# RUCAIBox/RecBole-CDR

Hardware: AMD Instinct MI355X
Metric: training interactions/sec (higher is better)
Workload: dtype f32; 1 GPU; C5: EMCDR-BPR D=128, 50000000 users x 10000000 items/domain (union tables 71.7 GB fp32), step = source batch + target batch of 1048576 triples each per rank, fwd+bwd+row-wise adam; batch_per_domain_per_rank=1048576, k_neg=1, optimizer=rowwise-adam

## Files before the change

recbole-cdr_amd/csrc/cdr_step.hip:

```cpp
#include <cstdlib>
#include <cstring>
#include <string.h>
#include <rocprim/device/device_radix_sort.hpp>
#include <rocprim/device/device_scan.hpp>
#include <rocprim/iterator/counting_iterator.hpp>
#include <rocprim/iterator/transform_iterator.hpp>
#include "cdr_common.h"
#include "cdr_adam_math.h"
#include "cdr_loss_math.h"

namespace {

constexpr int kUnroll = 4;

#ifndef CDR_NORM_REC_FLOATS
#define CDR_NORM_REC_FLOATS 16
#endif
constexpr int kNormRecFloats = CDR_NORM_REC_FLOATS;
static_assert(kNormRecFloats == 16 || kNormRecFloats == 32, "a record is one 64-byte or one 128-byte burst");

template <int LPR>
__device__ __forceinline__ float sqnorm4(float4 a) {
    if constexpr (LPR >= 32) {
        return __builtin_fmaf(a.w, a.w, __builtin_fmaf(a.z, a.z, __builtin_fmaf(a.x, a.x, a.y * a.y)));
// ... 246 lines not shown
        out6[6] = (float)acc[0]; out6[7] = (float)acc[1]; out6[8] = (float)acc[2];
    }
}

__global__ void finish_sums_kernel(const float* __restrict__ sums3, int64_t B, float reg_weight, float* __restrict__ out6) {
    if (threadIdx.x == 0 && blockIdx.x == 0) {
        const float main_loss = sums3[0] / (float)B;
        const float nu = sqrtf(sums3[1]), ni = sqrtf(sums3[2]);
        out6[1] = main_loss; out6[2] = nu; out6[3] = ni;
        out6[0] = main_loss + reg_weight * ((nu + ni) / (float)B);
        out6[4] = embloss_coef(reg_weight, B, nu);
        out6[5] = embloss_coef(reg_weight, B, ni);
    }
}

__global__ __launch_bounds__(kBlock) void make_keys_kernel(const int64_t* __restrict__ ids0, int64_t n0,
                                                           const int64_t* __restrict__ ids1, int64_t n1,
                                                           uint32_t* __restrict__ keys, uint32_t* __restrict__ vals) {
    const int64_t n = n0 + n1, stride = (int64_t)gridDim.x * kBlock;
    for (int64_t e = (int64_t)blockIdx.x * kBlock + threadIdx.x; e < n; e += stride) {
        keys[e] = (uint32_t)(e < n0 ? ids0[e] : ids1[e - n0]);
        vals[e] = (uint32_t)e;
    }
}

constexpr int kLongSeg = 32;
constexpr int kPiece = 256;

struct seg_long { int64_t head, len, base; };
struct seg_piece { int64_t start; int64_t len; };

struct apply_hp { float lr, b1, b2, eps, wd, step_size, bc2_sqrt; const float* dev; };
#define HP_FROM_DEV(h) do { if ((h).dev) { (h).step_size = (h).dev[0]; (h).bc2_sqrt = (h).dev[1]; } } while (0)
// ... 202 lines not shown
        if (NC) norm_rec_store<LPR>(n2 + (int64_t)row * kNormRecFloats, group_sum<LPR>(sqnorm4<LPR>(wnew)), sub);
    }
}
template <int LPR, int OPT>
__global__ __launch_bounds__(kBlock) void seg_long_finish_kernel(float* __restrict__ W, float* __restrict__ Mo, float* __restrict__ Vo,
                                                                 int D, const uint32_t* __restrict__ keys,
                                                                 const float* __restrict__ reg_coef, apply_hp hp,
                                                                 const unsigned* __restrict__ counters,
                                                                 const seg_long* __restrict__ longs,
                                                                 const float* __restrict__ partial, const int* __restrict__ pcnt) {
    seg_long_finish_body<LPR, OPT>(W, Mo, Vo, D, keys, reg_coef, hp, counters, longs, partial, pcnt);
}

__global__ __launch_bounds__(kBlock) void make_keys2_kernel(const int64_t* __restrict__ a, int64_t na, const int64_t* __restrict__ b0,
                                                            int64_t nb0, const int64_t* __restrict__ b1, int64_t nb1, uint32_t key_base,
                                                            uint32_t* __restrict__ keys, uint32_t* __restrict__ vals) {
    const int64_t n = na + nb0 + nb1, stride = (int64_t)gridDim.x * kBlock;
    for (int64_t e = (int64_t)blockIdx.x * kBlock + threadIdx.x; e < n; e += stride) {
        if (e < na) { keys[e] = (uint32_t)a[e]; vals[e] = (uint32_t)e; }
        else {
            const int64_t o = e - na;
            keys[e] = key_base + (uint32_t)(o < nb0 ? b0[o] : b1[o - nb0]);
            vals[e] = (uint32_t)o;
        }
    }
}


struct tab_ptrs { float* W; float* M; float* V; };

template <int OPT>
__device__ __forceinline__ float4 upd_math(float4 w, float4& m, float4& v, float4 acc, float rc, const apply_hp& h) {
    float4 gr = make_float4(acc.x + rc * w.x, acc.y + rc * w.y, acc.z + rc * w.z, acc.w + rc * w.w);
    if (h.wd != 0.f) { gr.x += h.wd * w.x; gr.y += h.wd * w.y; gr.z += h.wd * w.z; gr.w += h.wd * w.w; }
    if (OPT == 0) return make_float4(w.x - h.lr * gr.x, w.y - h.lr * gr.y, w.z - h.lr * gr.z, w.w - h.lr * gr.w);
    m.x += (gr.x - m.x) * (1.0f - h.b1); m.y += (gr.y - m.y) * (1.0f - h.b1);
    m.z += (gr.z - m.z) * (1.0f - h.b1); m.w += (gr.w - m.w) * (1.0f - h.b1);
    v.x = h.b2 * v.x + (1.0f - h.b2) * gr.x * gr.x; v.y = h.b2 * v.y + (1.0f - h.b2) * gr.y * gr.y;
    v.z = h.b2 * v.z + (1.0f - h.b2) * gr.z * gr.z; v.w = h.b2 * v.w + (1.0f - h.b2) * gr.w * gr.w;
// ... 172 lines not shown
        __syncthreads();
        unsigned sA = wbase[0][wave] + pA - cA, sB = wbase[1][wave] + pB - cB;
#pragma unroll
        for (int j = 0; j < kFlagIT; ++j) {
            if ((hA >> j) & 1u) headsA[sA++] = (uint32_t)(q0 + j);
            if ((hB >> j) & 1u) headsB[sB++] = (uint32_t)(q0 + j - nA);
        }
        __syncthreads();
    }
}

__global__ __launch_bounds__(kBlock) void coef_finish_kernel(const double* __restrict__ partials, int nblocks, int64_t B,
                                                             float reg_weight, float* __restrict__ out9, int kmul = 1,
                                                             int64_t* __restrict__ step_u_dev = nullptr, int64_t* __restrict__ step_i_dev = nullptr,
                                                             float* __restrict__ hp_dev = nullptr, float lr = 0.f, float b1 = 0.f, float b2 = 0.f,
                                                             unsigned* __restrict__ zero4 = nullptr, const float* __restrict__ norms2 = nullptr) {
    __shared__ double smem[2 * (kBlock / 64)];
    if (zero4 && threadIdx.x >= 64 && threadIdx.x < 68) zero4[threadIdx.x - 64] = 0u;
    if (hp_dev && threadIdx.x < 2) {
        int64_t* c = threadIdx.x == 0 ? step_u_dev : step_i_dev;
        const int64_t st = c[0] + 1;
        c[0] = st;
        cdr_adam_hp((double)st, lr, b1, b2, hp_dev[2 * threadIdx.x], hp_dev[2 * threadIdx.x + 1]);
    }
    double acc[2] = {0.0, 0.0};
    sum_partials<2, kBlock>(partials, nblocks, acc, smem);
    if (threadIdx.x == 0) {
        if (norms2) { acc[0] = (double)norms2[0]; acc[1] = (double)norms2[1]; }
        const float nu = (float)sqrt((double)kmul * acc[0]), ni = (float)sqrt((double)kmul * acc[1]);
        out9[4] = (reg_weight != 0.f && nu > 0.f) ? (float)kmul * (reg_weight / ((float)B * nu)) : 0.f;
        out9[5] = (reg_weight != 0.f && ni > 0.f) ? (float)kmul * (reg_weight / ((float)B * ni)) : 0.f;
    }
}
// ... 604 lines not shown
template <int LPR>
__global__ __launch_bounds__(kBlock) void seg_piece_sum2_kernel(int D, dup_side a, dup_side b) {
    const dup_side& t = blockIdx.y ? b : a;
    if (t.counters == nullptr) return;
    seg_piece_sum_body<LPR, true>(D, t.perm, t.G, t.neg_start, t.reg_limit, nullptr, t.counters, t.pieces, t.partial, t.pcnt);
}
template <int LPR, int OPT, bool NC = false>
__global__ __launch_bounds__(kBlock) void seg_long_finish2_kernel(int D, dup_side a, dup_side b) {
    const dup_side& t = blockIdx.y ? b : a;
    if (t.counters == nullptr) return;
    seg_long_finish_body<LPR, OPT, NC>(t.W, t.M, t.V, D, t.keys, t.reg_coef, t.hp, t.counters, t.longs, t.partial, t.pcnt, t.n2);
}

__global__ __launch_bounds__(kBlock) void shard_keys_kernel(const int64_t* __restrict__ recv3, int64_t Bl, uint32_t G, unsigned lb,
                                                            uint32_t key_base, int64_t* __restrict__ u_loc, uint32_t* __restrict__ keys,
                                                            uint32_t* __restrict__ vals, unsigned* __restrict__ cnt) {
    if (blockIdx.x == 0 && threadIdx.x < 4) cnt[threadIdx.x] = 0u;
    for (int64_t t = (int64_t)blockIdx.x * kBlock + threadIdx.x; t < Bl; t += (int64_t)gridDim.x * kBlock) {
        const int64_t u = recv3[3 * t];
        const uint32_t p = (uint32_t)recv3[3 * t + 1], n = (uint32_t)recv3[3 * t + 2];
        u_loc[t] = u;
        keys[t] = (uint32_t)u; vals[t] = (uint32_t)t;
        keys[Bl + t] = key_base + (((p % G) << lb) | (p / G)); vals[Bl + t] = (uint32_t)t;
        keys[2 * Bl + t] = key_base + (((n % G) << lb) | (n / G)); vals[2 * Bl + t] = (uint32_t)(Bl + t);
    }
}

struct head_flag_op {
    const uint32_t* keys;
    __device__ uint32_t operator()(uint32_t q) const { return (q == 0u || keys[q] != keys[q - 1]) ? 1u : 0u; }
};
// ... 527 lines not shown
    CDR_LAUNCH_CHECK();
    triplet_finish_kernel<<<dim3(1), dim3(kBlock), 0, s>>>(ctx->partials, grid, B, out3);
    CDR_LAUNCH_CHECK();
    return CDR_OK;
}

extern "C" int cdr_loss_finish_sums(void* stream, const float* sums3, int64_t B_mean, float reg_weight, float* out6) {
    CDR_CHECK_ARG(sums3 && out6 && B_mean > 0);
    finish_sums_kernel<<<dim3(1), dim3(64), 0, (hipStream_t)stream>>>(sums3, B_mean, reg_weight, out6);
    CDR_LAUNCH_CHECK();
    return CDR_OK;
}

using big_sort_config = rocprim::radix_sort_config<
    rocprim::default_config, rocprim::default_config,
    rocprim::radix_sort_onesweep_config<rocprim::kernel_config<1024, 8>, rocprim::kernel_config<1024, 8>, 9,
                                        rocprim::block_radix_rank_algorithm::match>,
    (size_t)1 << 17>;
constexpr int64_t kBigSort = 1 << 18;

static inline hipError_t sort_pairs(void* tmp, size_t& tmp_bytes, const uint32_t* kin, uint32_t* kout, const uint32_t* vin, uint32_t* vout,
                                    size_t n, unsigned bits, hipStream_t s) {
    if ((int64_t)n >= kBigSort) return rocprim::radix_sort_pairs<big_sort_config>(tmp, tmp_bytes, kin, kout, vin, vout, n, 0u, bits, s);
    return rocprim::radix_sort_pairs(tmp, tmp_bytes, kin, kout, vin, vout, n, 0u, bits, s);
}

static inline unsigned bits_for(int64_t num_rows) {
    unsigned b = 1;
    while (b < 32 && ((int64_t)1 << b) < num_rows) ++b;
    return b;
}

namespace {

inline size_t up256(size_t b) { return (b + 255) & ~(size_t)255; }

struct heads_view {
    unsigned* cnt; uint32_t* headsA; uint32_t* headsB;
    heads_view(uint32_t* heads, int64_t n_a) : cnt((unsigned*)heads), headsA(heads + 4), headsB(headsA + (n_a / 2 + 1)) {}
    static int64_t words(int64_t n_a, int64_t n_b) { return 4 + (n_a / 2 + 1) + (n_b / 2 + 1); }
};

inline size_t count_list_bytes(int64_t B) {
    int64_t P = 1024;
    while (P < 3 * B) P <<= 1;
    return (size_t)(P + kListHdr) * sizeof(uint64_t);
// ... 24 lines not shown
        o_part = o_cnt + up256(sizeof(int) * piece_cap); bytes = o_part + sizeof(float) * (size_t)piece_cap * D;
    }
    void bind(char* base, dup_side& t) const {
        t.counters = (unsigned*)base; t.longs = (seg_long*)(base + o_long); t.pieces = (seg_piece*)(base + o_piece);
        t.pcnt = (int*)(base + o_cnt); t.partial = (float*)(base + o_part);
    }
};

}

extern "C" int cdr_sort_workspace_bytes(int64_t n, int64_t num_rows, size_t* bytes) {
    CDR_CHECK_ARG(bytes && n > 0 && num_rows > 0 && num_rows <= (int64_t)0xFFFFFFFFu && n <= (int64_t)0x7FFFFFFF);
    size_t tmp = 0;
    hipError_t e = sort_pairs(nullptr, tmp, nullptr, nullptr, nullptr, nullptr, (size_t)n, bits_for(num_rows), (hipStream_t)0);
    if (e != hipSuccess) { cdr_set_error("cdr_sort_workspace_bytes: %s", hipGetErrorString(e)); return (int)e; }
    *bytes = up256(tmp) + 2 * up256((size_t)n * sizeof(uint32_t));
    return CDR_OK;
}

template <class MakeKeys>
static int sort_ids_with(cdr_ctx* ctx, hipStream_t s, int64_t n, int64_t key_space, uint32_t* keys_sorted, uint32_t* perm, void* ws,
                         size_t ws_bytes, MakeKeys&& make_keys) {
    size_t need = 0;
    int rc = cdr_sort_workspace_bytes(n, key_space, &need);
    if (rc) return rc;
    CDR_CHECK_ARG(ws_bytes >= need);
    const size_t arr = up256((size_t)n * sizeof(uint32_t));
    uint32_t* keys_in = (uint32_t*)ws;
    uint32_t* vals_in = (uint32_t*)((char*)ws + arr);
    void* tmp = (char*)ws + 2 * arr;
    size_t tmp_bytes = ws_bytes - 2 * arr;
    cdr_time_scope ts(ctx, CDR_TAG_SORT, s);
    make_keys(keys_in, vals_in);
    CDR_LAUNCH_CHECK();
    CDR_HIP(sort_pairs(tmp, tmp_bytes, keys_in, keys_sorted, vals_in, perm, (size_t)n, bits_for(key_space), s));
    return CDR_OK;
}

extern "C" int cdr_sort_ids(cdr_ctx* ctx, void* stream, const int64_t* ids0, int64_t n0, const int64_t* ids1, int64_t n1,
                            int64_t num_rows, uint32_t* keys_sorted, uint32_t* perm, void* workspace,
                            size_t workspace_bytes) {
    const int64_t n = n0 + n1;
    CDR_CHECK_ARG(ids0 && n0 > 0 && (n1 == 0 || ids1) && keys_sorted && perm && workspace);
    hipStream_t s = (hipStream_t)stream;
    return sort_ids_with(ctx, s, n, num_rows, keys_sorted, perm, workspace, workspace_bytes, [&](uint32_t* keys_in, uint32_t* vals_in) {
        make_keys_kernel<<<dim3(grid_for(n, kBlock)), dim3(kBlock), 0, s>>>(ids0, n0, ids1, n1, keys_in, vals_in);
    });
}

extern "C" int cdr_sort_ids_two_tables(cdr_ctx* ctx, void* stream, const int64_t* ids_a, int64_t n_a, int64_t rows_a,
                                       const int64_t* ids_b0, int64_t n_b0, const int64_t* ids_b1, int64_t n_b1, int64_t rows_b,
                                       uint32_t* keys_sorted, uint32_t* perm, uint32_t* key_base_out, void* workspace,
                                       size_t workspace_bytes) {
    const int64_t n = n_a + n_b0 + n_b1;
    CDR_CHECK_ARG(ids_a && n_a > 0 && ids_b0 && n_b0 > 0 && (n_b1 == 0 || ids_b1) && keys_sorted && perm && key_base_out && workspace);
    CDR_CHECK_ARG(rows_a > 0 && rows_b > 0);
    const unsigned hb = two_table_bits(rows_a, rows_b);
    CDR_CHECK_ARG(hb < 31);
    const uint32_t key_base = 1u << hb;
    hipStream_t s = (hipStream_t)stream;
    int rc = sort_ids_with(ctx, s, n, (int64_t)key_base * 2, keys_sorted, perm, workspace, workspace_bytes, [&](uint32_t* keys_in, uint32_t* vals_in) {
        make_keys2_kernel<<<dim3(grid_for(n, kBlock)), dim3(kBlock), 0, s>>>(ids_a, n_a, ids_b0, n_b0, ids_b1, n_b1, key_base, keys_in, vals_in);
    });
    if (rc) return rc;
    *key_base_out = key_base;
    return CDR_OK;
}

extern "C" int cdr_rowwise_apply(cdr_ctx* ctx, void* stream, int opt, float* table, float* exp_avg, float* exp_avg_sq, int D,
                                 const uint32_t* keys_sorted, const uint32_t* perm, int64_t n, const float* G,
                                 int64_t neg_start, int64_t reg_limit, const float* reg_coef, float lr, float beta1,
                                 float beta2, float eps, float weight_decay, int64_t step, const int64_t* occ_ids, uint32_t key_base) {
    CDR_CHECK_ARG(table && keys_sorted && perm && G && n > 0);
    CDR_CHECK_ARG(D > 0 && (D & 3) == 0);
    CDR_CHECK_ARG(opt == 0 || (opt == 1 && exp_avg && exp_avg_sq && step > 0));
    hipStream_t s = (hipStream_t)stream;
    if (key_base) {
        table -= (int64_t)key_base * D;
        if (exp_avg) exp_avg -= (int64_t)key_base * D;
        if (exp_avg_sq) exp_avg_sq -= (int64_t)key_base * D;
    }
// ... 33 lines not shown
    return CDR_OK;
}

namespace {

struct step_tables { tab_ptrs TU, TI; apply_hp hu, hi; };
step_tables make_tables(int opt_user, float* user_tab, float* user_m, float* user_v, int64_t step_user, int opt_item, float* item_tab,
                        float* item_m, float* item_v, int64_t step_item, float lr, float beta1, float beta2, float eps, float wd) {
    return {{user_tab, user_m, user_v}, {item_tab, item_m, item_v}, make_hp(opt_user, lr, beta1, beta2, eps, wd, step_user),
            make_hp(opt_item, lr, beta1, beta2, eps, wd, step_item)};
}

int embloss_head(cdr_ctx* ctx, hipStream_t s, const float* user_tab, const float* item_tab, int D, const int64_t* uid, const int64_t* pid,
                 int64_t n_rows, int64_t B, int kmul, float reg_weight, float* out9, unsigned* cnt, int64_t* step_user_dev = nullptr,
                 int64_t* step_item_dev = nullptr, float* hp_dev = nullptr, float lr = 0.f, float beta1 = 0.f, float beta2 = 0.f,
                 const float* user_n2 = nullptr, const float* item_n2 = nullptr) {
    int ngrid = 0;
    if (reg_weight != 0.f) {
        const int lpr = cdr_lpr_for(D);
        ngrid = grid_for((n_rows + 7) / 8, kBlock / lpr);
        cdr_time_scope ts(ctx, CDR_TAG_BATCH_NORMS, s);
        if (user_n2 && item_n2) {
            DISPATCH_LPR(lpr, batch_norms_cached_kernel<L><<<dim3(ngrid), dim3(kBlock), 0, s>>>(user_n2, item_n2, uid, pid, n_rows, ctx->partials));
        } else {
            DISPATCH_LPR(lpr, batch_norms_kernel<L><<<dim3(ngrid), dim3(kBlock), 0, s>>>(user_tab, item_tab, D, uid, pid, n_rows, ctx->partials));
        }
        CDR_LAUNCH_CHECK();
    }
    coef_finish_kernel<<<dim3(1), dim3(kBlock), 0, s>>>(ctx->partials, ngrid, B, ngrid ? reg_weight : 0.f, out9, kmul, step_user_dev, step_item_dev, hp_dev,
                                                        lr, beta1, beta2, cnt);
    CDR_LAUNCH_CHECK();
    return CDR_OK;
}

int occ_flags(cdr_ctx* ctx, hipStream_t s, const uint32_t* keys, const uint32_t* perm, int64_t n_a, int64_t n, int fstride, uint8_t* flags,
              const heads_view& hv, bool stat = false) {
    cdr_time_scope ts(ctx, CDR_TAG_OCC_FLAGS, s);
    occ_flags_kernel<<<dim3(grid_for(n, kBlock * kFlagIT)), dim3(kBlock), 0, s>>>(keys, perm, n_a, n, fstride, flags, hv.headsA, hv.headsB, hv.cnt, stat);
    CDR_LAUNCH_CHECK();
    return CDR_OK;
}

struct dup_host { tab_ptrs T; const uint32_t* keys; const uint32_t* perm; int64_t n; const uint32_t* heads; const unsigned* nheads;
                  const float* G; int64_t neg_start, reg_limit; const float* reg_coef; apply_hp hp; uint32_t key_base;
                  float* out = nullptr; const uint32_t* uidx = nullptr; float* n2 = nullptr; };
// ... 119 lines not shown
        }
        CDR_LAUNCH_CHECK();
        coef_finish_kernel<<<dim3(1), dim3(kBlock), 0, s>>>(ctx->partials, reg_weight != 0.f ? ngrid : 0, B, reg_weight, out9, 1, step_user_dev, step_item_dev, hp_dev,
                                                            lr, beta1, beta2, hv.cnt);
        CDR_LAUNCH_CHECK();
        {
            cdr_time_scope ts(ctx, CDR_TAG_OCC_FLAGS, s);
            count_flags_kernel<<<dim3(grid_for(B, kBlock)), dim3(kBlock), 0, s>>>(uid, pid, nid, B, ctx->idc_user, ctx->idc_item, key_base, (uint32_t*)flags,
                                                                                 (uint64_t*)ctx->idc_list, hv.cnt);
            CDR_LAUNCH_CHECK();
            count_sort_kernel<<<dim3(kRankBlocks + 128), dim3(1024), 0, s>>>(uid, pid, nid, B, ctx->idc_user, ctx->idc_item, key_base,
                                                                                            (uint64_t*)ctx->idc_list, keys, perm, hv.headsA, hv.headsB, hv.cnt);
        }
        CDR_LAUNCH_CHECK();
    } else {
        rc = embloss_head(ctx, s, user_tab, item_tab, D, uid, pid, B, B, 1, reg_weight, out9, hv.cnt, step_user_dev, step_item_dev, hp_dev, lr, beta1, beta2,
                          NU, NI);
        if (rc) return rc;
        rc = cdr_sort_ids_two_tables(ctx, stream, uid, B, user_rows, pid, B, nid, B, item_rows, keys, perm, &key_base, sort_ws, sort_ws_bytes);
        if (rc) return rc;
        rc = occ_flags(ctx, s, keys, perm, B, 3 * B, 4, flags, hv, B <= kCountMaxB);
        if (rc) return rc;
    }
    step_tables T = make_tables(opt, user_tab, user_m, user_v, step_user, opt, item_tab, item_m, item_v, step_item, lr, beta1, beta2, eps, weight_decay);
    if (hp_dev && opt == 1) { T.hu.dev = hp_dev; T.hi.dev = hp_dev + 2; }
    static const int un = [] { const char* e = getenv("CDR_FWD_APPLY_UN"); return (e && e[0] == '2') ? 2 : 1; }();
    const int grid = grid_for((B + un - 1) / un, kBlock / lpr);
    {
        cdr_time_scope ts(ctx, CDR_TAG_BPR_FWD_APPLY, s);
        DISPATCH_LPR_OPT(lpr, opt, {
            constexpr int U2 = O == 1 ? 2 : 1;
            auto kern = cached ? (un == 2 ? bpr_fwd_apply_kernel<L, O, U2, false, false, true> : bpr_fwd_apply_kernel<L, O, 1, false, false, true>)
                               : (un == 2 ? bpr_fwd_apply_kernel<L, O, U2> : bpr_fwd_apply_kernel<L, O, 1>);
            kern<<<dim3(grid), dim3(kBlock), 0, s>>>(T.TU, T.TI, D, uid, pid, nid, (const uint32_t*)flags, B, gamma, 1.0f / (float)B, out9 + 4, T.hu, T.hi, GU, GP,
// ... 312 lines not shown
extern "C" int cdr_bpr_shard_plan(cdr_ctx* ctx, void* stream, const int64_t* recv3, int64_t Bl, int64_t user_rows, int64_t item_local_rows,
                                  int world, int64_t* u_loc, uint32_t* keys, uint32_t* perm, uint8_t* flags, uint32_t* heads,
                                  uint32_t* uidx, int64_t* uniq_local, int64_t* umap, int64_t* counts, int64_t* n_uniq, void* ws,
                                  size_t ws_bytes) {
    CDR_CHECK_ARG(ctx && recv3 && u_loc && keys && perm && flags && heads && uidx && uniq_local && umap && counts && n_uniq && ws);
    CDR_CHECK_ARG(Bl > 0 && 3 * Bl <= (int64_t)0x7FFFFFFF && ((uintptr_t)flags & 3) == 0);
    shard_bits kb;
    CDR_CHECK_ARG(shard_key_bits(user_rows, item_local_rows, world, kb) == CDR_OK);
    size_t scan_need = 0;
    int rc = shard_scan_bytes(Bl, &scan_need);
    if (rc) return rc;
    CDR_CHECK_ARG(ws_bytes >= scan_need);
    hipStream_t s = (hipStream_t)stream;
    const int64_t n = 3 * Bl;
    const heads_view hv(heads, Bl);
    rc = sort_ids_with(ctx, s, n, (int64_t)kb.key_base * 2, keys, perm, ws, ws_bytes, [&](uint32_t* keys_in, uint32_t* vals_in) {
        shard_keys_kernel<<<dim3(grid_for(Bl, kBlock)), dim3(kBlock), 0, s>>>(recv3, Bl, (uint32_t)world, kb.lb, kb.key_base, u_loc, keys_in, vals_in, hv.cnt);
    });
    if (rc) return rc;
    rc = occ_flags(ctx, s, keys, perm, Bl, n, 4, flags, hv);
    if (rc) return rc;
    const int64_t nB = 2 * Bl;
    const uint32_t* keysB = keys + Bl;
    const size_t arrB = up256((size_t)nB * sizeof(uint32_t));
    uint32_t* excl = (uint32_t*)ws;
    void* stmp = (char*)ws + arrB;
    size_t stmp_bytes = ws_bytes - arrB;
    CDR_HIP(rocprim::exclusive_scan(stmp, stmp_bytes, rocprim::make_transform_iterator(rocprim::make_counting_iterator<uint32_t>(0u), head_flag_op{keysB}),
                                    excl, 0u, (size_t)nB, rocprim::plus<uint32_t>(), s));
    shard_emit_kernel<<<dim3(grid_for(nB, kBlock)), dim3(kBlock), 0, s>>>(keysB, perm + Bl, excl, nB, world, kb.lb, kb.key_base, uidx, uniq_local, umap,
                                                                          counts, n_uniq);
    CDR_LAUNCH_CHECK();
// ... 112 lines not shown
        });
    }
    CDR_LAUNCH_CHECK();
    dup_host sides[2];
    make_sides(sides, T, keys, perm, hv, GU, GI, S, nI, nI, S, out9 + 4, out9 + 5, key_base);
    return finish_and_apply_dups(ctx, s, opt, D, sides, [&](unsigned* za, unsigned* zb) {
        step_finish_keep_kernel<<<dim3(1), dim3(kBlock), 0, s>>>(ctx->partials, grid, B, reg_weight, out9, za, zb);
    });
}

namespace {

__global__ __launch_bounds__(kBlock) void make_keys_pair_kernel(const int64_t* __restrict__ a0, int64_t na0, const int64_t* __restrict__ a1,
                                                                int64_t na1, const int64_t* __restrict__ b0, int64_t nb0,
                                                                const int64_t* __restrict__ b1, int64_t nb1, uint32_t key_base,
                                                                uint32_t* __restrict__ keys, uint32_t* __restrict__ vals) {
    const int64_t na = na0 + na1, n = na + nb0 + nb1, stride = (int64_t)gridDim.x * kBlock;
    for (int64_t e = (int64_t)blockIdx.x * kBlock + threadIdx.x; e < n; e += stride) {
        if (e < na) { keys[e] = (uint32_t)(e < na0 ? a0[e] : a1[e - na0]); vals[e] = (uint32_t)e; }
        else {
            const int64_t o = e - na;
            keys[e] = key_base + (uint32_t)(o < nb0 ? b0[o] : b1[o - nb0]);
            vals[e] = (uint32_t)o;
        }
    }
}

template <int LPR>
__global__ __launch_bounds__(kBlock) void pair_norms_kernel(const float* __restrict__ U, const float* __restrict__ I, int D,
                                                            const int64_t* __restrict__ su, const int64_t* __restrict__ si, int64_t Bs,
                                                            const int64_t* __restrict__ tu, const int64_t* __restrict__ ti, int64_t Bt,
// ... 180 lines not shown
    const float wreg_s = alpha * reg_s, wreg_t = (1.0f - alpha) * reg_t;
    const heads_view hv(heads, N);
    int ngrid = 0;
    if (wreg_s != 0.f || wreg_t != 0.f) {
        ngrid = grid_for((N + 7) / 8, kBlock / lpr);
        cdr_time_scope ts(ctx, CDR_TAG_BATCH_NORMS, s);
        DISPATCH_LPR(lpr, pair_norms_kernel<L><<<dim3(ngrid), dim3(kBlock), 0, s>>>(user_tab, item_tab, D, su, si, B_s, tu, ti, B_t, ctx->partials));
        CDR_LAUNCH_CHECK();
    }
    pair_coef_kernel<<<dim3(1), dim3(kBlock), 0, s>>>(ctx->partials, ngrid, B_s, B_t, wreg_s, wreg_t, out16, step_user_dev, step_item_dev,
                                                      opt == 1 ? hp_dev : nullptr, lr, beta1, beta2, hv.cnt);
    CDR_LAUNCH_CHECK();
    const unsigned hb = two_table_bits(user_rows, item_rows);
    CDR_CHECK_ARG(hb < 31);
    const uint32_t key_base = 1u << hb;
    int rc = sort_ids_with(ctx, s, 2 * N, (int64_t)key_base * 2, keys, perm, sort_ws, sort_ws_bytes, [&](uint32_t* keys_in, uint32_t* vals_in) {
        make_keys_pair_kernel<<<dim3(grid_for(2 * N, kBlock)), dim3(kBlock), 0, s>>>(su, B_s, tu, B_t, si, B_s, ti, B_t, key_base, keys_in, vals_in);
    });
    if (rc) return rc;
    rc = occ_flags(ctx, s, keys, perm, N, 2 * N, 4, flags, hv);
    if (rc) return rc;
    step_tables T = make_tables(opt, user_tab, user_m, user_v, 1, opt, item_tab, item_m, item_v, 1, lr, beta1, beta2, eps, weight_decay);
    if (opt == 1) { T.hu.dev = hp_dev; T.hi.dev = hp_dev + 2; }
    const int grid = grid_for(N, kBlock / lpr);
    {
        cdr_time_scope ts(ctx, CDR_TAG_POINT_FWD_GRAD, s);
        DISPATCH_LPR_OPT(lpr, opt, point_pair_fwd_apply_kernel<L, O><<<dim3(grid), dim3(kBlock), 0, s>>>(
                                       loss_kind, T.TU, T.TI, D, su, si, ys, B_s, tu, ti, yt, B_t, (const uint32_t*)flags, alpha / (float)B_s, (1.0f - alpha) / (float)B_t,
                                       out16 + 9, T.hu, T.hi, GU, GI, ctx->partials));
    }
    CDR_LAUNCH_CHECK();
    dup_host sides[2];
// ... 6 lines not shown
```

Baseline: 568.7 million interactions/s.

## Replace rocPRIM sort driver with own onesweep passes and fuse setup into key kernels

For large sorts with rocPRIM 4.2, the change stops calling rocPRIM's sort_pairs wrapper and launches rocPRIM's onesweep histogram, scan and pass device functions directly. The clearing of sort workspace state (lookback, block ids, counts) moves into the key-building kernels, or into the coefficient-finish kernel. On the two-table path, the digit histogram and its prefix scan are folded into the key-generation kernel. The aim is to drop memset, histogram and scan launches and one extra read of the keys per step. The price is reliance on rocPRIM detail internals tied to one version, plus more shared-memory atomics in the key kernel.

```diff
diff --git a/recbole-cdr_amd/csrc/cdr_step.hip b/recbole-cdr_amd/csrc/cdr_step.hip
--- a/recbole-cdr_amd/csrc/cdr_step.hip
+++ b/recbole-cdr_amd/csrc/cdr_step.hip
@@ -284,9 +284,16 @@
     }
 }
 
+__device__ __forceinline__ void sort_state_clear(uint32_t* __restrict__ zspan, int64_t zwords) {
+    if (!zspan) return;
+    for (int64_t i = (int64_t)blockIdx.x * blockDim.x + threadIdx.x; i < zwords; i += (int64_t)gridDim.x * blockDim.x) zspan[i] = 0u;
+}
+
 __global__ __launch_bounds__(kBlock) void make_keys_kernel(const int64_t* __restrict__ ids0, int64_t n0,
                                                            const int64_t* __restrict__ ids1, int64_t n1,
-                                                           uint32_t* __restrict__ keys, uint32_t* __restrict__ vals) {
+                                                           uint32_t* __restrict__ keys, uint32_t* __restrict__ vals,
+                                                           uint32_t* __restrict__ zspan, int64_t zwords) {
+    sort_state_clear(zspan, zwords);
     const int64_t n = n0 + n1, stride = (int64_t)gridDim.x * kBlock;
     for (int64_t e = (int64_t)blockIdx.x * kBlock + threadIdx.x; e < n; e += stride) {
         keys[e] = (uint32_t)(e < n0 ? ids0[e] : ids1[e - n0]);
@@ -519,7 +526,9 @@
 
 __global__ __launch_bounds__(kBlock) void make_keys2_kernel(const int64_t* __restrict__ a, int64_t na, const int64_t* __restrict__ b0,
                                                             int64_t nb0, const int64_t* __restrict__ b1, int64_t nb1, uint32_t key_base,
-                                                            uint32_t* __restrict__ keys, uint32_t* __restrict__ vals) {
+                                                            uint32_t* __restrict__ keys, uint32_t* __restrict__ vals,
+                                                            uint32_t* __restrict__ zspan, int64_t zwords) {
+    sort_state_clear(zspan, zwords);
     const int64_t n = na + nb0 + nb1, stride = (int64_t)gridDim.x * kBlock;
     for (int64_t e = (int64_t)blockIdx.x * kBlock + threadIdx.x; e < n; e += stride) {
         if (e < na) { keys[e] = (uint32_t)a[e]; vals[e] = (uint32_t)e; }
@@ -528,6 +537,64 @@
             keys[e] = key_base + (uint32_t)(o < nb0 ? b0[o] : b1[o - nb0]);
             vals[e] = (uint32_t)o;
         }
+    }
+}
+
+constexpr unsigned kSortBlock = 1024, kSortItems = 8, kSortRadixBits = 9, kSortRadix = 1u << kSortRadixBits;
+constexpr unsigned kSortMaxPlaces = (32 + kSortRadixBits - 1) / kSortRadixBits;
+using sort_offs_t = size_t;
+
+__global__ __launch_bounds__(kSortBlock) void make_keys2_offsets_kernel(const int64_t* __restrict__ a, int64_t na, const int64_t* __restrict__ b0,
+                                                                        int64_t nb0, const int64_t* __restrict__ b1, int64_t nb1,
+                                                                        uint32_t key_base, uint32_t* __restrict__ keys, uint32_t* __restrict__ vals,
+                                                                        uint32_t* __restrict__ zspan, int64_t zwords,
+                                                                        sort_offs_t* __restrict__ counts, unsigned* __restrict__ ticket, unsigned places) {
+    constexpr unsigned kStripes = 4;
+    __shared__ unsigned hist[kSortMaxPlaces * kSortRadix * kStripes];
+    sort_state_clear(zspan, zwords);
+    const unsigned tid = threadIdx.x, bins = places * kSortRadix;
+    for (unsigned i = tid; i < bins * kStripes; i += kSortBlock) hist[i] = 0u;
+    __syncthreads();
+    const unsigned stripe = tid % kStripes;
+    const int64_t n = na + nb0 + nb1, stride = (int64_t)gridDim.x * kSortBlock;
+    for (int64_t e = (int64_t)blockIdx.x * kSortBlock + tid; e < n; e += stride) {
+        uint32_t k, v;
+        if (e < na) { k = (uint32_t)a[e]; v = (uint32_t)e; }
+        else {
+            const int64_t o = e - na;
+            k = key_base + (uint32_t)(o < nb0 ? b0[o] : b1[o - nb0]);
+            v = (uint32_t)o;
+        }
+        keys[e] = k; vals[e] = v;
+        for (unsigned p = 0; p < places; ++p) {
+            const unsigned digit = (k >> (p * kSortRadixBits)) & (kSortRadix - 1u);
+            atomicAdd(&hist[(p * kSortRadix + digit) * kStripes + stripe], 1u);
+        }
+    }
+    __syncthreads();
+    for (unsigned i = tid; i < bins; i += kSortBlock) {
+        unsigned t = 0;
+#pragma unroll
+        for (unsigned j = 0; j < kStripes; ++j) t += hist[i * kStripes + j];
+        if (t) atomicAdd(reinterpret_cast<unsigned long long*>(counts + i), (unsigned long long)t);
+    }
+    if (!cdr_sign_in_last(ticket, gridDim.x)) return;
+    unsigned* sc = hist;
+    for (unsigned p = 0; p < places; ++p) {
+        unsigned c = 0;
+        if (tid < kSortRadix) {
+            c = (unsigned)__hip_atomic_load(reinterpret_cast<unsigned long long*>(counts + p * kSortRadix + tid), __ATOMIC_RELAXED, __HIP_MEMORY_SCOPE_AGENT);
+            sc[tid] = c;
+        }
+        __syncthreads();
+        for (unsigned d = 1; d < kSortRadix; d <<= 1) {
+            const unsigned t = (tid < kSortRadix && tid >= d) ? sc[tid - d] : 0u;
+            __syncthreads();
+            if (tid < kSortRadix) sc[tid] += t;
+            __syncthreads();
+        }
+        if (tid < kSortRadix) counts[p * kSortRadix + tid] = (sort_offs_t)(sc[tid] - c);
+        __syncthreads();
     }
 }
 
@@ -730,9 +797,13 @@
                                                              float reg_weight, float* __restrict__ out9, int kmul = 1,
                                                              int64_t* __restrict__ step_u_dev = nullptr, int64_t* __restrict__ step_i_dev = nullptr,
                                                              float* __restrict__ hp_dev = nullptr, float lr = 0.f, float b1 = 0.f, float b2 = 0.f,
-                                                             unsigned* __restrict__ zero4 = nullptr, const float* __restrict__ norms2 = nullptr) {
+                                                             unsigned* __restrict__ zero4 = nullptr, const float* __restrict__ norms2 = nullptr,
+                                                             uint32_t* __restrict__ zspan = nullptr, int zwords = 0) {
     __shared__ double smem[2 * (kBlock / 64)];
     if (zero4 && threadIdx.x >= 64 && threadIdx.x < 68) zero4[threadIdx.x - 64] = 0u;
+    if (zspan) {
+        for (int i = threadIdx.x; i < zwords; i += kBlock) zspan[i] = 0u;
+    }
     if (hp_dev && threadIdx.x < 2) {
         int64_t* c = threadIdx.x == 0 ? step_u_dev : step_i_dev;
         const int64_t st = c[0] + 1;
@@ -1367,7 +1438,9 @@
 
 __global__ __launch_bounds__(kBlock) void shard_keys_kernel(const int64_t* __restrict__ recv3, int64_t Bl, uint32_t G, unsigned lb,
                                                             uint32_t key_base, int64_t* __restrict__ u_loc, uint32_t* __restrict__ keys,
-                                                            uint32_t* __restrict__ vals, unsigned* __restrict__ cnt) {
+                                                            uint32_t* __restrict__ vals, unsigned* __restrict__ cnt,
+                                                            uint32_t* __restrict__ zspan, int64_t zwords) {
+    sort_state_clear(zspan, zwords);
     if (blockIdx.x == 0 && threadIdx.x < 4) cnt[threadIdx.x] = 0u;
     for (int64_t t = (int64_t)blockIdx.x * kBlock + threadIdx.x; t < Bl; t += (int64_t)gridDim.x * kBlock) {
         const int64_t u = recv3[3 * t];
@@ -1925,7 +1998,7 @@
 
 using big_sort_config = rocprim::radix_sort_config<
     rocprim::default_config, rocprim::default_config,
-    rocprim::radix_sort_onesweep_config<rocprim::kernel_config<1024, 8>, rocprim::kernel_config<1024, 8>, 9,
+    rocprim::radix_sort_onesweep_config<rocprim::kernel_config<kSortBlock, kSortItems>, rocprim::kernel_config<kSortBlock, kSortItems>, kSortRadixBits,
                                         rocprim::block_radix_rank_algorithm::match>,
     (size_t)1 << 17>;
 constexpr int64_t kBigSort = 1 << 18;
@@ -1941,6 +2014,92 @@
     while (b < 32 && ((int64_t)1 << b) < num_rows) ++b;
     return b;
 }
+
+#if ROCPRIM_VERSION == 400200
+#define CDR_HAVE_OWN_SORT 1
+namespace {
+
+namespace rpd = rocprim::detail;
+using sort_bid_t = rpd::block_id_wrapper<unsigned int, true>;
+
+__global__ __launch_bounds__(kSortBlock) void sort_hist_kernel(const uint32_t* keys, sort_offs_t* counts, sort_offs_t size, sort_offs_t full_blocks,
+                                                               unsigned end_bit) {
+    rpd::onesweep_histograms<kSortBlock, kSortItems, kSortRadixBits, false>(keys, counts, size, full_blocks, rocprim::identity_decomposer{}, 0u, end_bit);
+}
+__global__ __launch_bounds__(kSortBlock) void sort_scan_kernel(sort_offs_t* counts) {
+    rpd::onesweep_scan_histograms<kSortBlock, kSortRadixBits>(counts);
+}
+__global__ __launch_bounds__(kSortBlock) void sort_pass_kernel(const uint32_t* keys_in, uint32_t* keys_out, const uint32_t* vals_in, uint32_t* vals_out,
+                                                               unsigned size, sort_offs_t* offs_in, sort_offs_t* offs_out,
+                                                               rpd::onesweep_lookback_state* lookback, unsigned bit, unsigned cur_bits,
+                                                               unsigned full_blocks, sort_bid_t bid) {
+    rpd::onesweep_iteration<kSortBlock, kSortItems, kSortRadixBits, false, rocprim::block_radix_rank_algorithm::match>(
+        keys_in, keys_out, vals_in, vals_out, size, offs_in, offs_out, lookback, rocprim::identity_decomposer{}, bit, cur_bits, full_blocks, bid);
+}
+
+struct own_sort_plan {
+    unsigned blocks = 0, full_blocks = 0, places = 0;
+    int64_t wordsA = 0, wordsB = 0;
+    size_t o_ids = 0, o_lookback = 0, o_offs_tmp = 0, o_keys_tmp = 0, o_vals_tmp = 0, bytes = 0;
+    own_sort_plan(size_t n, unsigned bits) {
+        constexpr size_t per_block = (size_t)kSortBlock * kSortItems;
+        blocks = (unsigned)((n + per_block - 1) / per_block);
+        full_blocks = n % per_block == 0 ? blocks : blocks - 1;
+        places = (bits + kSortRadixBits - 1) / kSortRadixBits;
+        const size_t arr = ((n * sizeof(uint32_t)) + 255) & ~(size_t)255;
+        wordsA = (int64_t)(places * kSortRadix * (sizeof(sort_offs_t) / 4) + 32);
+        o_ids = (size_t)wordsA * 4;
+        o_lookback = o_ids + (size_t)kSortMaxPlaces * 128;
+        const size_t lb_bytes = (size_t)places * blocks * kSortRadix * sizeof(rpd::onesweep_lookback_state);
+        wordsB = (int64_t)((o_lookback + lb_bytes - o_ids) / 4);
+        o_offs_tmp = (o_lookback + lb_bytes + 255) & ~(size_t)255;
+        o_keys_tmp = o_offs_tmp + kSortRadix * sizeof(sort_offs_t);
+        o_vals_tmp = o_keys_tmp + arr;
+        bytes = o_vals_tmp + arr;
+    }
+    sort_offs_t* counts(char* tmp) const { return (sort_offs_t*)tmp; }
+    unsigned* ticket(char* tmp) const { return (unsigned*)(tmp + (size_t)wordsA * 4 - 128); }
+};
+static_assert(sizeof(rpd::onesweep_lookback_state) == 4 && sizeof(sort_offs_t) % 4 == 0, "the zero span is counted in 32-bit words");
+
+constexpr int64_t kOwnSortMax = (int64_t)1 << 30;
+
+inline bool own_sort_on(int64_t n) {
+    static const bool on = [] { const char* e = getenv("CDR_OWN_SORT"); return !(e && e[0] == '0'); }();
+    return on && n >= kBigSort && n <= kOwnSortMax;
+}
+
+inline hipError_t own_sort_offsets(const own_sort_plan& P, char* tmp, const uint32_t* keys_in, size_t n, unsigned bits, hipStream_t s) {
+    sort_hist_kernel<<<dim3(P.blocks), dim3(kSortBlock), 0, s>>>(keys_in, P.counts(tmp), (sort_offs_t)n, (sort_offs_t)P.full_blocks, bits);
+    sort_scan_kernel<<<dim3(P.places), dim3(kSortBlock), 0, s>>>(P.counts(tmp));
+    return hipGetLastError();
+}
+
+inline hipError_t own_sort_passes(const own_sort_plan& P, char* tmp, const uint32_t* keys_in, uint32_t* keys_out, const uint32_t* vals_in,
+                                  uint32_t* vals_out, size_t n, unsigned bits, hipStream_t s) {
+    uint32_t* keys_tmp = (uint32_t*)(tmp + P.o_keys_tmp);
+    uint32_t* vals_tmp = (uint32_t*)(tmp + P.o_vals_tmp);
+    auto* lookback = (rpd::onesweep_lookback_state*)(tmp + P.o_lookback);
+    bool to_output = (P.places - 1) % 2 == 0, from_input = true;
+    unsigned place = 0;
+    for (unsigned bit = 0; bit < bits; bit += kSortRadixBits, ++place) {
+        const uint32_t* ki = from_input ? keys_in : (to_output ? keys_tmp : keys_out);
+        const uint32_t* vi = from_input ? vals_in : (to_output ? vals_tmp : vals_out);
+        const unsigned cur_bits = bits - bit < kSortRadixBits ? bits - bit : kSortRadixBits;
+        sort_pass_kernel<<<dim3(P.blocks), dim3(kSortBlock), 0, s>>>(
+            ki, to_output ? keys_out : keys_tmp, vi, to_output ? vals_out : vals_tmp, (unsigned)n, P.counts(tmp) + (size_t)place * kSortRadix,
+            (sort_offs_t*)(tmp + P.o_offs_tmp), lookback + (size_t)place * P.blocks * kSortRadix, bit, cur_bits, P.full_blocks,
+            sort_bid_t::create(tmp + P.o_ids + (size_t)place * 128));
+        from_input = false;
+        to_output = !to_output;
+    }
+    return hipGetLastError();
+}
+
+}
+#else
+#define CDR_HAVE_OWN_SORT 0
+#endif
 
 namespace {
 
@@ -1995,13 +2154,21 @@
     size_t tmp = 0;
     hipError_t e = sort_pairs(nullptr, tmp, nullptr, nullptr, nullptr, nullptr, (size_t)n, bits_for(num_rows), (hipStream_t)0);
     if (e != hipSuccess) { cdr_set_error("cdr_sort_workspace_bytes: %s", hipGetErrorString(e)); return (int)e; }
+#if CDR_HAVE_OWN_SORT
+    if (n >= kBigSort && n <= kOwnSortMax) {
+        const size_t own = own_sort_plan((size_t)n, bits_for(num_rows)).bytes;
+        if (own > tmp) tmp = own;
+    }
+#endif
     *bytes = up256(tmp) + 2 * up256((size_t)n * sizeof(uint32_t));
     return CDR_OK;
 }
 
+struct sort_clear { uint32_t* p; int64_t words; };
+
 template <class MakeKeys>
 static int sort_ids_with(cdr_ctx* ctx, hipStream_t s, int64_t n, int64_t key_space, uint32_t* keys_sorted, uint32_t* perm, void* ws,
-                         size_t ws_bytes, MakeKeys&& make_keys) {
+                         size_t ws_bytes, MakeKeys&& make_keys, bool keys_make_offsets = false) {
     size_t need = 0;
     int rc = cdr_sort_workspace_bytes(n, key_space, &need);
     if (rc) return rc;
@@ -2009,14 +2176,41 @@
     const size_t arr = up256((size_t)n * sizeof(uint32_t));
     uint32_t* keys_in = (uint32_t*)ws;
     uint32_t* vals_in = (uint32_t*)((char*)ws + arr);
-    void* tmp = (char*)ws + 2 * arr;
+    char* tmp = (char*)ws + 2 * arr;
     size_t tmp_bytes = ws_bytes - 2 * arr;
+    const unsigned bits = bits_for(key_space);
     cdr_time_scope ts(ctx, CDR_TAG_SORT, s);
-    make_keys(keys_in, vals_in);
+#if CDR_HAVE_OWN_SORT
+    if (own_sort_on(n)) {
+        CDR_CHECK_ARG(((uintptr_t)tmp & 127) == 0);
+        const own_sort_plan P((size_t)n, bits);
+        if (keys_make_offsets) {
+            make_keys(keys_in, vals_in, sort_clear{(uint32_t*)(tmp + P.o_ids), P.wordsB});
+            CDR_LAUNCH_CHECK();
+        } else {
+            make_keys(keys_in, vals_in, sort_clear{(uint32_t*)tmp, P.wordsA + P.wordsB});
+            CDR_LAUNCH_CHECK();
+            CDR_HIP(own_sort_offsets(P, tmp, keys_in, (size_t)n, bits, s));
+        }
+        CDR_HIP(own_sort_passes(P, tmp, keys_in, keys_sorted, vals_in, perm, (size_t)n, bits, s));
+        return CDR_OK;
+    }
+#endif
+    make_keys(keys_in, vals_in, sort_clear{nullptr, 0});
     CDR_LAUNCH_CHECK();
-    CDR_HIP(sort_pairs(tmp, tmp_bytes, keys_in, keys_sorted, vals_in, perm, (size_t)n, bits_for(key_space), s));
+    CDR_HIP(sort_pairs(tmp, tmp_bytes, keys_in, keys_sorted, vals_in, perm, (size_t)n, bits, s));
     return CDR_OK;
 }
+
+#if CDR_HAVE_OWN_SORT
+static sort_clear own_sort_span_a(int64_t n, int64_t key_space, void* ws, size_t ws_bytes) {
+    size_t need = 0;
+    if (!own_sort_on(n) || cdr_sort_workspace_bytes(n, key_space, &need) != CDR_OK || ws_bytes < need) return {nullptr, 0};
+    return {(uint32_t*)((char*)ws + 2 * up256((size_t)n * sizeof(uint32_t))), own_sort_plan((size_t)n, bits_for(key_space)).wordsA};
+}
+#else
+static sort_clear own_sort_span_a(int64_t, int64_t, void*, size_t) { return {nullptr, 0}; }
+#endif
 
 extern "C" int cdr_sort_ids(cdr_ctx* ctx, void* stream, const int64_t* ids0, int64_t n0, const int64_t* ids1, int64_t n1,
                             int64_t num_rows, uint32_t* keys_sorted, uint32_t* perm, void* workspace,
@@ -2024,28 +2218,46 @@
     const int64_t n = n0 + n1;
     CDR_CHECK_ARG(ids0 && n0 > 0 && (n1 == 0 || ids1) && keys_sorted && perm && workspace);
     hipStream_t s = (hipStream_t)stream;
-    return sort_ids_with(ctx, s, n, num_rows, keys_sorted, perm, workspace, workspace_bytes, [&](uint32_t* keys_in, uint32_t* vals_in) {
-        make_keys_kernel<<<dim3(grid_for(n, kBlock)), dim3(kBlock), 0, s>>>(ids0, n0, ids1, n1, keys_in, vals_in);
+    return sort_ids_with(ctx, s, n, num_rows, keys_sorted, perm, workspace, workspace_bytes, [&](uint32_t* keys_in, uint32_t* vals_in, sort_clear z) {
+        make_keys_kernel<<<dim3(grid_for(n, kBlock)), dim3(kBlock), 0, s>>>(ids0, n0, ids1, n1, keys_in, vals_in, z.p, z.words);
     });
+}
+
+static inline uint32_t two_table_key_base(int64_t rows_a, int64_t rows_b) {
+    const unsigned hb = two_table_bits(rows_a, rows_b);
+    return hb < 31 ? 1u << hb : 0u;
+}
+
+static int sort_two_tables(cdr_ctx* ctx, void* stream, const int64_t* ids_a, int64_t n_a, int64_t rows_a, const int64_t* ids_b0,
+                           int64_t n_b0, const int64_t* ids_b1, int64_t n_b1, int64_t rows_b, uint32_t* keys_sorted, uint32_t* perm,
+                           uint32_t* key_base_out, void* workspace, size_t workspace_bytes, sort_clear span_a) {
+    const int64_t n = n_a + n_b0 + n_b1;
+    CDR_CHECK_ARG(ids_a && n_a > 0 && ids_b0 && n_b0 > 0 && (n_b1 == 0 || ids_b1) && keys_sorted && perm && key_base_out && workspace);
+    CDR_CHECK_ARG(rows_a > 0 && rows_b > 0);
+    const uint32_t key_base = two_table_key_base(rows_a, rows_b);
+    CDR_CHECK_ARG(key_base != 0u);
+    hipStream_t s = (hipStream_t)stream;
+    int rc = sort_ids_with(ctx, s, n, (int64_t)key_base * 2, keys_sorted, perm, workspace, workspace_bytes, [&](uint32_t* keys_in, uint32_t* vals_in, sort_clear z) {
+        if (span_a.p && z.p) {
+            const unsigned places = (bits_for((int64_t)key_base * 2) + kSortRadixBits - 1) / kSortRadixBits;
+            const unsigned kgrid = (unsigned)((n + (int64_t)kSortBlock * kSortItems - 1) / ((int64_t)kSortBlock * kSortItems));
+            make_keys2_offsets_kernel<<<dim3(kgrid), dim3(kSortBlock), 0, s>>>(ids_a, n_a, ids_b0, n_b0, ids_b1, n_b1, key_base, keys_in, vals_in, z.p, z.words,
+                                                                               (sort_offs_t*)span_a.p, (unsigned*)span_a.p + span_a.words - 32, places);
+        } else {
+            make_keys2_kernel<<<dim3(grid_for(n, kBlock)), dim3(kBlock), 0, s>>>(ids_a, n_a, ids_b0, n_b0, ids_b1, n_b1, key_base, keys_in, vals_in, z.p, z.words);
+        }
+    }, span_a.p != nullptr);
+    if (rc) return rc;
+    *key_base_out = key_base;
+    return CDR_OK;
 }
 
 extern "C" int cdr_sort_ids_two_tables(cdr_ctx* ctx, void* stream, const int64_t* ids_a, int64_t n_a, int64_t rows_a,
                                        const int64_t* ids_b0, int64_t n_b0, const int64_t* ids_b1, int64_t n_b1, int64_t rows_b,
                                        uint32_t* keys_sorted, uint32_t* perm, uint32_t* key_base_out, void* workspace,
                                        size_t workspace_bytes) {
-    const int64_t n = n_a + n_b0 + n_b1;
-    CDR_CHECK_ARG(ids_a && n_a > 0 && ids_b0 && n_b0 > 0 && (n_b1 == 0 || ids_b1) && keys_sorted && perm && key_base_out && workspace);
-    CDR_CHECK_ARG(rows_a > 0 && rows_b > 0);
-    const unsigned hb = two_table_bits(rows_a, rows_b);
-    CDR_CHECK_ARG(hb < 31);
-    const uint32_t key_base = 1u << hb;
-    hipStream_t s = (hipStream_t)stream;
-    int rc = sort_ids_with(ctx, s, n, (int64_t)key_base * 2, keys_sorted, perm, workspace, workspace_bytes, [&](uint32_t* keys_in, uint32_t* vals_in) {
-        make_keys2_kernel<<<dim3(grid_for(n, kBlock)), dim3(kBlock), 0, s>>>(ids_a, n_a, ids_b0, n_b0, ids_b1, n_b1, key_base, keys_in, vals_in);
-    });
-    if (rc) return rc;
-    *key_base_out = key_base;
-    return CDR_OK;
+    return sort_two_tables(ctx, stream, ids_a, n_a, rows_a, ids_b0, n_b0, ids_b1, n_b1, rows_b, keys_sorted, perm, key_base_out, workspace,
+                           workspace_bytes, sort_clear{nullptr, 0});
 }
 
 extern "C" int cdr_rowwise_apply(cdr_ctx* ctx, void* stream, int opt, float* table, float* exp_avg, float* exp_avg_sq, int D,
@@ -2109,7 +2321,7 @@
 int embloss_head(cdr_ctx* ctx, hipStream_t s, const float* user_tab, const float* item_tab, int D, const int64_t* uid, const int64_t* pid,
                  int64_t n_rows, int64_t B, int kmul, float reg_weight, float* out9, unsigned* cnt, int64_t* step_user_dev = nullptr,
                  int64_t* step_item_dev = nullptr, float* hp_dev = nullptr, float lr = 0.f, float beta1 = 0.f, float beta2 = 0.f,
-                 const float* user_n2 = nullptr, const float* item_n2 = nullptr) {
+                 const float* user_n2 = nullptr, const float* item_n2 = nullptr, sort_clear zspan = {nullptr, 0}) {
     int ngrid = 0;
     if (reg_weight != 0.f) {
         const int lpr = cdr_lpr_for(D);
@@ -2123,7 +2335,7 @@
         CDR_LAUNCH_CHECK();
     }
     coef_finish_kernel<<<dim3(1), dim3(kBlock), 0, s>>>(ctx->partials, ngrid, B, ngrid ? reg_weight : 0.f, out9, kmul, step_user_dev, step_item_dev, hp_dev,
-                                                        lr, beta1, beta2, cnt);
+                                                        lr, beta1, beta2, cnt, nullptr, zspan.p, (int)zspan.words);
     CDR_LAUNCH_CHECK();
     return CDR_OK;
 }
@@ -2273,10 +2485,13 @@
         }
         CDR_LAUNCH_CHECK();
     } else {
+        static const bool keys_make_offsets = [] { const char* e = getenv("CDR_OWN_SORT"); return !(e && e[0] == '1'); }();
+        const uint32_t kb = two_table_key_base(user_rows, item_rows);
+        const sort_clear span_a = keys_make_offsets && kb ? own_sort_span_a(3 * B, (int64_t)kb * 2, sort_ws, sort_ws_bytes) : sort_clear{nullptr, 0};
         rc = embloss_head(ctx, s, user_tab, item_tab, D, uid, pid, B, B, 1, reg_weight, out9, hv.cnt, step_user_dev, step_item_dev, hp_dev, lr, beta1, beta2,
-                          NU, NI);
+                          NU, NI, span_a);
         if (rc) return rc;
-        rc = cdr_sort_ids_two_tables(ctx, stream, uid, B, user_rows, pid, B, nid, B, item_rows, keys, perm, &key_base, sort_ws, sort_ws_bytes);
+        rc = sort_two_tables(ctx, stream, uid, B, user_rows, pid, B, nid, B, item_rows, keys, perm, &key_base, sort_ws, sort_ws_bytes, span_a);
         if (rc) return rc;
         rc = occ_flags(ctx, s, keys, perm, B, 3 * B, 4, flags, hv, B <= kCountMaxB);
         if (rc) return rc;
@@ -2619,8 +2834,9 @@
     hipStream_t s = (hipStream_t)stream;
     const int64_t n = 3 * Bl;
     const heads_view hv(heads, Bl);
-    rc = sort_ids_with(ctx, s, n, (int64_t)kb.key_base * 2, keys, perm, ws, ws_bytes, [&](uint32_t* keys_in, uint32_t* vals_in) {
-        shard_keys_kernel<<<dim3(grid_for(Bl, kBlock)), dim3(kBlock), 0, s>>>(recv3, Bl, (uint32_t)world, kb.lb, kb.key_base, u_loc, keys_in, vals_in, hv.cnt);
+    rc = sort_ids_with(ctx, s, n, (int64_t)kb.key_base * 2, keys, perm, ws, ws_bytes, [&](uint32_t* keys_in, uint32_t* vals_in, sort_clear z) {
+        shard_keys_kernel<<<dim3(grid_for(Bl, kBlock)), dim3(kBlock), 0, s>>>(recv3, Bl, (uint32_t)world, kb.lb, kb.key_base, u_loc, keys_in, vals_in, hv.cnt,
+                                                                             z.p, z.words);
     });
     if (rc) return rc;
     rc = occ_flags(ctx, s, keys, perm, Bl, n, 4, flags, hv);
@@ -2763,7 +2979,9 @@
 __global__ __launch_bounds__(kBlock) void make_keys_pair_kernel(const int64_t* __restrict__ a0, int64_t na0, const int64_t* __restrict__ a1,
                                                                 int64_t na1, const int64_t* __restrict__ b0, int64_t nb0,
                                                                 const int64_t* __restrict__ b1, int64_t nb1, uint32_t key_base,
-                                                                uint32_t* __restrict__ keys, uint32_t* __restrict__ vals) {
+                                                                uint32_t* __restrict__ keys, uint32_t* __restrict__ vals,
+                                                                uint32_t* __restrict__ zspan, int64_t zwords) {
+    sort_state_clear(zspan, zwords);
     const int64_t na = na0 + na1, n = na + nb0 + nb1, stride = (int64_t)gridDim.x * kBlock;
     for (int64_t e = (int64_t)blockIdx.x * kBlock + threadIdx.x; e < n; e += stride) {
         if (e < na) { keys[e] = (uint32_t)(e < na0 ? a0[e] : a1[e - na0]); vals[e] = (uint32_t)e; }
@@ -2974,8 +3192,8 @@
     const unsigned hb = two_table_bits(user_rows, item_rows);
     CDR_CHECK_ARG(hb < 31);
     const uint32_t key_base = 1u << hb;
-    int rc = sort_ids_with(ctx, s, 2 * N, (int64_t)key_base * 2, keys, perm, sort_ws, sort_ws_bytes, [&](uint32_t* keys_in, uint32_t* vals_in) {
-        make_keys_pair_kernel<<<dim3(grid_for(2 * N, kBlock)), dim3(kBlock), 0, s>>>(su, B_s, tu, B_t, si, B_s, ti, B_t, key_base, keys_in, vals_in);
+    int rc = sort_ids_with(ctx, s, 2 * N, (int64_t)key_base * 2, keys, perm, sort_ws, sort_ws_bytes, [&](uint32_t* keys_in, uint32_t* vals_in, sort_clear z) {
+        make_keys_pair_kernel<<<dim3(grid_for(2 * N, kBlock)), dim3(kBlock), 0, s>>>(su, B_s, tu, B_t, si, B_s, ti, B_t, key_base, keys_in, vals_in, z.p, z.words);
     });
     if (rc) return rc;
     rc = occ_flags(ctx, s, keys, perm, N, 2 * N, 4, flags, hv);
```

After: 580.6 million interactions/s (median of 6 runs). +2.1%, better.
